# slowkow/scde

Measured on AMD Instinct MI355X. Metric: genes/sec for scde.expression.difference (400-pt grid, 100 randomizations), higher is better.
Workload: dtype f64; 1 GPU; config3: synthetic 20000 genes x 1000 cells (500/500), 401-pt grid, 100 bootstraps, n.cores=1 seeding; genes_total=20000, genes_per_gpu=20000, cells=1000, grid=401, n_randomizations=100, parallelism=gene-shard x1 (strong)

## Files before the change

scde_amd/csrc/engine.hip:

```cpp
#include <hip/hip_runtime.h>

#include <algorithm>
#include <chrono>
#include <cfloat>
#include <cmath>
#include <cerrno>
#include <cstdarg>
#include <cstdio>
#include <cstdlib>
#include <cstring>
#include <condition_variable>
#include <deque>
#include <functional>
#include <thread>
#include <atomic>
#include <memory>
#include <unistd.h>
#include <mutex>
#include <numeric>
#include <string>
#include <vector>

#include "engine_internal.h"
#include "kernels.h"
// ... 691 lines not shown
      pu.into_col0 = col0;
      pu.into_c0 = c0;
      pu.into_cap_hint = c0 > 0 ? (long long)((double)col0 / c0 * C * 1.1) : 0;
      const PostSpec* sp[1] = {&ps};
      UniqueSet* up[1] = {&pu};
      const hipStream_t main = cx->stream;
      cx->stream = s.piece_stream;
      const int rc = build_unique_sets(cx, sp, up, 1);
      cx->stream = main;
      pu.into = nullptr;
      RCHK(rc);
      HCHK(handoff_spin(cx, s.piece_stream));
      HCHK(hipEventRecord(s.piece_ev[j], s.piece_stream));
      HCHK(handoff_wait(cx, st, s.piece_ev[j]));
      for (int c = c0; c < c1; ++c) ucl_off_h[c + 1] = col0 + pu.ucl_off_h[c - c0 + 1];
      const long long nc = pu.ucl_off_h[c1 - c0];
      if (j == jlast) RCHK(upload(cx, u.ucl_off, ucl_off_h.data(), sizeof(long long) * (C + 1)));
      const long long est = std::max<long long>(col0 + nc, (long long)((double)(col0 + nc) / c1 * C * 1.1));
      RCHK(setup_tables(plan0, est, j > 0));
      RCHK(launch_tables_range(plan0, c0, c1, col0, pu.ucl_off.as<long long>(), pu.ucl_off_h, j == jlast, pu));
      if (modes_pieces) {
        HCHK(launch_modes(u.uci.as<int>() + (size_t)N * c0, N, N, c1 - c0, pu.ucl_off.as<long long>(),
                          cx->maxi.as<int>() + col0, cx->mag.as<double>(), s.modes + (size_t)N * c0, 1, N, st));
        const size_t bytes = sizeof(double) * (size_t)N * (c1 - c0);
        RCHK(dnl_push(cx, st, s.modes_host + (size_t)N * c0, bytes, s.modes + (size_t)N * c0, bytes, bytes, 1));
      }
      col0 += nc;
    }
    ta.ucl_off = u.ucl_off.as<long long>();
    tables_done = make_plan(col0) == plan0;
  }
  const long long ncols = ucl_off_h[C];
  const Plan plan = make_plan(ncols);
  const bool fast = plan.fast, fused = plan.fused, stretch_skip = plan.stretch_skip;
  bool tpath = plan.tpath;
  ta.ncols = ncols;
  if (!tables_done) {
    if (plan.tpath && !plan0.tpath) {
      HCHK(cx->qflags.ensure(sizeof(int) * 40));
      HCHK(hipMemsetAsync(cx->qflags.p, 0, sizeof(int) * 40, st));
    }
    if (plan.fused) {
      HCHK(cx->base_col.ensure(sizeof(int) * std::max(1, C)));
      HCHK(cx->zcol.ensure(sizeof(int) * std::max(1, C)));
    }
    RCHK(setup_tables(plan, ncols, false));
    ta.ncols = ncols;
    RCHK(launch_tables_range(plan, 0, C, 0, u.ucl_off.as<long long>(), ucl_off_h, true, cx->task_us));
  }
  std::vector<int> draws;
  std::vector<double> W;
  int ndraw = 0, maxw = 0;
  const int nsets = (int)s.seeds.size();
  const int qstride = (int)round_up(std::max(Cmax, 1), 64) + 64;
  int nb = fast ? boot2_nb(s.nboot) : 16;
  if (fast) {
    const int v = cx->opt_boot_nb;
    if (v >= 4 && v <= 32 && v % 4 == 0) nb = v;
  }
  const int Bp = (int)round_up(std::max(s.nboot, 1), nb);
  const int Bt = (int)round_up(Bp, 32) + 128;
  auto rest_fn = [=, &s, &u]() mutable -> int {
  if (want_modes && s.modes && s.modes_early && !modes_pieces) {
    HCHK(launch_modes(u.uci.as<int>(), N, N, C, u.ucl_off.as<long long>(), cx->maxi.as<int>(),
                      cx->mag.as<double>(), s.modes, 1, N, st));
    if (s.modes_host) {
      const size_t bytes = sizeof(double) * (size_t)N * C;
      RCHK(dnl_push(cx, st, s.modes_host, bytes, s.modes, bytes, bytes, 1));
    } else {
      if (!cx->modes_ev) HCHK(hipEventCreateWithFlags(&cx->modes_ev, hipEventDisableTiming));
      HCHK(handoff_spin(cx, st));
      HCHK(hipEventRecord(cx->modes_ev, st));
    }
  }
  bool jp_sent = false;
  const bool dev_mult = fused && C <= kMultMaxCells;
  if (fused && s.nboot > 0) {
    if (dev_mult) {
      make_draws(s, Bp, draws, W, ndraw, &maxw, false);
    } else {
      make_draws(s, Bp, draws, W, ndraw);
      maxw = 0;
      for (double w : W) maxw = std::max(maxw, (int)w);
    }
    tpath = tpath && maxw <= std::min(127, cx->opt_tile_max_mult);
  }
  if (!s.batch_call && s.ensemble) {
    HCHK(cx->E.ensure(sizeof(double) * std::max<long long>(1, ncols) * GS));
    HCHK(launch_ensemble_cols(cx->T.as<double>(), ncols, G, GS, cx->E.as<double>(), st));
    NoBootArgs na{cx->E.as<double>(), G, GS, u.ucl_off.as<long long>(), u.uci.as<int>(), N, C, N, 1,
                  s.jp, s.jp_g, s.jp_k};
    HCHK(launch_noboot(na, st));
  } else if (s.nboot == 0 && !s.batch_call) {
    NoBootArgs na{cx->T.as<double>(), G, GS, u.ucl_off.as<long long>(), u.uci.as<int>(), N, C, N, 0,
                  s.jp, s.jp_g, s.jp_k};
    HCHK(launch_noboot(na, st));
  } else if (s.nboot == 0) {
    HCHK(hipMemsetAsync(s.jp, 0, sizeof(double) * (size_t)N * G, st));
  } else {
    if (!fused) make_draws(s, Bp, draws, W, ndraw);
    hipStream_t sa = st;
    if (fused) {
      if (!cx->aux_stream) HCHK(hipStreamCreateWithFlags(&cx->aux_stream, hipStreamNonBlocking));
      if (!cx->aux_ev) HCHK(hipEventCreateWithFlags(&cx->aux_ev, hipEventDisableTiming));
      sa = cx->aux_stream;
      HCHK(handoff_wait(cx, sa, cx->p1_ev));
// ... 1938 lines not shown
```

scde_amd/csrc/kernels.h:

```cpp
#pragma once

#ifndef SCDE_BOOT_WPE
#define SCDE_BOOT_WPE 8
#endif
#ifndef SCDE_BOOT_ASMLD
#define SCDE_BOOT_ASMLD 1
#endif
#ifndef SCDE_TAB_WPE
#define SCDE_TAB_WPE 4
#endif
#ifndef SCDE_BOOT_EB
#define SCDE_BOOT_EB 4
#endif
#ifndef SCDE_BOOT_DIAG
#define SCDE_BOOT_DIAG 0
#endif
#ifndef SCDE_RATIO_WPE
#define SCDE_RATIO_WPE 1
#endif
#ifndef SCDE_RATIO_DIAG
#define SCDE_RATIO_DIAG 0
#endif
#ifndef SCDE_WPCA_BLOCK
#define SCDE_WPCA_BLOCK 512
// ... 133 lines not shown
  const long long* ucl_off;
  const int* uci;
  long long ld_uci;
  double norm_mult;
  const int* degen;
  double* out;
  long long out_g, out_k;
  int ngenes;
  int g_lo = 0, g_hi = -1;
};

struct NoBootArgs {
  const double* T;
  int G, GS;
  const long long* ucl_off;
  const int* uci;
  long long ld_uci;
  int ncells, ngenes;
  int ensemble;
  double* out;
  long long out_g, out_k;
};

struct RatioArgs {
  const double* jp1;
  long long j1g, j1k;
  const double* jp2;
  long long j2g, j2k;
  const double* prior_y;
  int n, ngenes;
  int normalize;
  const double* xin;
  long long xg, xo;
  double* ratio;
  long long rg, ro;
  const double* diffv;
  int zi;
  double* res;
  long long res_ld;
};

hipError_t launch_cell_prep(const double* models, int ncells, int G, int GS, const double* mag, int lt, int sq,
                            double* mu, double* lcfp, double* lcfpr, double* theta, double* cellscal,
                            double* pq, hipStream_t s, double* cfp = nullptr);
hipError_t launch_col_consts(const int* ucl, const long long* ucl_off, long long ncols, int ncells,
                             const double* theta, int GS, const double* cellscal, double* colc, hipStream_t s);
hipError_t launch_tables(const TablesArgs& a, hipStream_t s);
hipError_t launch_stretch_zu(const double* U, const int* base_col, int ncells, const double* Wt, int Bp, int nsets,
                             double* ZU, hipStream_t s, int gsets = 0, int gsplit = 0);
hipError_t launch_base_cols(const int* ucl, const long long* ucl_off, int ncells, const unsigned char* has_clamp,
                            int use_baseline, int* base_col, hipStream_t s);
hipError_t launch_widen16(const unsigned short* in, int* out, size_t n, hipStream_t s);
hipError_t launch_patch32(const int2* exc, size_t n, int* out, hipStream_t s);
hipError_t launch_ell(const int* uci, long long ld_uci, int ngenes, int ncells, const long long* ucl_off,
                      const int* base_col, int stride, int pad_col, int padto, int2* ent, int* nnz, hipStream_t s,
                      int cell_off, const int* ucl = nullptr, unsigned* key = nullptr, int* idx = nullptr,
                      int kg0 = 0, int kgn = 0, int kch = 1, int desc = 0);
hipError_t launch_baseline_z(const double* T, int G, int GS, const int* base_col, int ncells, const double* Wt,
                             int Bp, int nsets, double* Z, hipStream_t s, int gsets = 0, int gsplit = 0);
constexpr int kMultMaxCells = 16384;
hipError_t launch_mult(const int* draws, int nsets, int nboot, int ndraw, int ncells, int Bp, double* Wt, int Bt,
                       unsigned char* W8, int nb, int P, unsigned char* W8p, int SG, int NGR, unsigned char* W8g,
                       hipStream_t s);
hipError_t launch_spin(hipStream_t s, long long cycles);
hipError_t launch_boot(const BootArgs& a, hipStream_t s);
hipError_t launch_boot_exact(const ExactArgs& a, hipStream_t s);
int boot2_nb(int nboot);
hipError_t launch_boot2(const Boot2Args& a, hipStream_t s);
hipError_t launch_delta(const double* T, const long long* ucl_off, int ncells, long long ncols, const int* base_col,
                        int G, int GS, double* D, hipStream_t s);
hipError_t launch_noboot(const NoBootArgs& a, hipStream_t s);
hipError_t launch_ensemble_cols(const double* T, long long ncols, int G, int GS, double* E, hipStream_t s);
hipError_t launch_modes(const int* uci, long long ld_uci, int ngenes, int ncells, const long long* ucl_off,
                        const int* maxi, const double* mag, double* modes, long long mg, long long mc,
                        hipStream_t s);
hipError_t launch_post(const int* uci, long long ld_uci, int ngenes, int c, const long long* ucl_off,
                       const double* T, int G, int GS, double* post, long long pg, long long pk, hipStream_t s);
hipError_t launch_cell_minmax(const int* counts, long long ld, long long g0, int ngenes, int ncells,
                              const int* cellidx, int* cmax, int* cmin, hipStream_t s);
hipError_t launch_mark(const int* counts, long long ld, long long g0, int ngenes, int ncells, const int* cellidx,
                       const long long* woff, unsigned long long* bits, hipStream_t s,
                       int* flags = nullptr);
hipError_t launch_rank(const unsigned long long* bits, const long long* woff, int ncells, int* rank, int* nuniq,
                       hipStream_t s,
                       const int* flags_in = nullptr, int* flags_out = nullptr);
hipError_t launch_fill_ucl(const unsigned long long* bits, const long long* woff, int ncells, const int* rank,
                           const long long* ucl_off, int* ucl, hipStream_t s);
hipError_t launch_uci(const int* counts, long long ld, long long g0, int ngenes, int ncells, const int* cellidx,
                      const long long* woff, const unsigned long long* bits, const int* rank, int* uci,
                      hipStream_t s);
hipError_t launch_colmajor_to_rows(const double* src, int nrows, int ncols, int GS, double* dst, hipStream_t s);
hipError_t launch_bh_cz(const double* z, int n, double* cz, void* work, size_t* work_bytes, hipStream_t s);

hipError_t launch_prior_stats(const int* counts, long long ld, int N, int C, const double* cellp, int sq,
                              double* vout, int* occ, double* partials, int nb, double* out, hipStream_t s);
long long prior_items(int N, int C);
int prior_blocks(int N, int C, int cap);
int prior_grid_n(int L);
hipError_t launch_prior_bin(const int* counts, long long ld, int N, int C, const double* cellp, int sq,
                            const int* occ, double wsum, double max_value, double bw, int L,
                            unsigned long long* hist, int nb, hipStream_t s);
hipError_t launch_prior_tail(double tot_mass, double max_value, double bw, int L, double pc,
                             const unsigned long long* hist, double* work, double* out, hipStream_t s);
hipError_t launch_sort_doubles(const double* in, double* out, long long n, void* work, size_t* work_bytes,
                               hipStream_t s);
hipError_t launch_ratio_summary(const RatioArgs& a, hipStream_t s);
// ... 172 lines not shown
```

scde_amd/csrc/kernels.hip:

```cpp
#include <hip/hip_runtime.h>
#include <algorithm>
#include <cmath>
#include <cstdint>
#include <utility>

#include "device_math.h"
#include "kernels.h"
#include "wave_ops.h"

namespace scde {

__global__ __launch_bounds__(256) void k_cell_prep(const double* __restrict__ models, int ncells, int G, int GS,
                                                   const double* __restrict__ mag, int localtheta,
                                                   int squarelogit, double* __restrict__ mu,
                                                   double* __restrict__ lcfp, double* __restrict__ lcfpr,
                                                   double* __restrict__ theta, double* __restrict__ cellscal,
                                                   double* __restrict__ pq, double* __restrict__ cfpo) {
  const int c = blockIdx.x;
  auto M = [&](int col) { return models[(long long)c + (long long)ncells * col]; };
  const double concb = M(0), conca = M(1), failr = M(2), corrb = M(3), corra = M(4), corrt = M(5);
  const double ltb = M(6), ltt = M(7), ltm = M(8), lts = M(9), ltr = M(10), conca2 = M(11);
  double lmax = -INFINITY;
  for (int k = threadIdx.x; k < G; k += blockDim.x) {
    const double m = mag[k];
// ... 1676 lines not shown
    const unsigned qv[16] = {q0.x, q0.y, q0.z, q0.w, q1.x, q1.y, q1.z, q1.w,
                             q2.x, q2.y, q2.z, q2.w, q3.x, q3.y, q3.z, q3.w};
#pragma unroll
    for (int tt = 0; tt < 16; ++tt) sq[tt * 64 + lane] = qv[tt];
    const unsigned wv[8] = {w0.x, w0.y, w0.z, w0.w, w1.x, w1.y, w1.z, w1.w};
    unsigned short* sw16 = reinterpret_cast<unsigned short*>(sw);
#pragma unroll
    for (int j = 0; j < 8; ++j) {
      sw16[(2 * j) * 64 + lane] = (unsigned short)(wv[j] & 0xffffu);
      sw16[(2 * j + 1) * 64 + lane] = (unsigned short)(wv[j] >> 16);
    }
    wave_sync();
    const uint4* bq = reinterpret_cast<const uint4*>(sq + t * 64 + 16 * h);
    const uint4 b0v = bq[0], b1v = bq[1], b2v = bq[2], b3v = bq[3];
    const unsigned u[16] = {b0v.x, b0v.y, b0v.z, b0v.w, b1v.x, b1v.y, b1v.z, b1v.w,
                            b2v.x, b2v.y, b2v.z, b2v.w, b3v.x, b3v.y, b3v.z, b3v.w};
    const uint4* aw = reinterpret_cast<const uint4*>(sw + r * 32 + 8 * h);
    const uint4 a0v = aw[0], a1v = aw[1];
    const unsigned x2[8] = {a0v.x, a0v.y, a0v.z, a0v.w, a1v.x, a1v.y, a1v.z, a1v.w};
    i32x4 af[2];
    unsigned lo4[4], hi4[4];
#pragma unroll
    for (int q = 0; q < 4; ++q) {
      lo4[q] = __builtin_amdgcn_perm(x2[2 * q + 1], x2[2 * q], 0x06040200u);
      hi4[q] = __builtin_amdgcn_perm(x2[2 * q + 1], x2[2 * q], 0x07050301u);
    }
    af[0] = i32x4{(int)lo4[0], (int)lo4[1], (int)lo4[2], (int)lo4[3]};
    af[1] = i32x4{(int)hi4[0], (int)hi4[1], (int)hi4[2], (int)hi4[3]};
    unsigned pl[4][4];
#pragma unroll
    for (int q = 0; q < 4; ++q)
      tr4(u[4 * q], u[4 * q + 1], u[4 * q + 2], u[4 * q + 3], pl[0][q], pl[1][q], pl[2][q], pl[3][q]);
#pragma unroll
    for (int l = 0; l < 4; ++l) {
      const i32x4 bf = {(int)pl[l][0], (int)pl[l][1], (int)pl[l][2], (int)pl[l][3]};
      acc[0][l] = mfma_i8(af[0], bf, acc[0][l]);
      acc[1][l] = mfma_i8(af[1], bf, acc[1][l]);
    }
  }
  if (t < NTB)
#pragma unroll
    for (int bt = 0; bt < 2; ++bt)
#pragma unroll
      for (int q = 0; q < 4; ++q) {
        const int b = 16 * bt + 4 * h + q;
        if (b < nbout) {
          const long long v =
              (((long long)acc[bt][3][q] * 256 + acc[bt][2][q]) * 256 + acc[bt][1][q]) * 256 + acc[bt][0][q];
          atomicAdd(reinterpret_cast<unsigned long long*>(&dsum[t * 32 + b]), (unsigned long long)v);
        }
      }
}

template <int NB>
__device__ __forceinline__ void tile_rows(double (&a0)[NB], double (&a1)[NB], const double* __restrict__ D,
                                          const int2* __restrict__ E, int n, const double* __restrict__ W,
                                          const double* __restrict__ Zs, int GS, int Bp, int b0, int k0, int r,
                                          bool live, bool l0, bool l1) {
#pragma unroll
  for (int i = 0; i < NB; ++i) {
    const d2_t z = live ? *reinterpret_cast<const d2_t*>(Zs + (long long)(b0 + i) * GS + k0) : d2_t{0.0, 0.0};
    a0[i] = l0 ? z.x : -INFINITY;
    a1[i] = l1 ? z.y : -INFINITY;
  }
  {
    constexpr int EB2 = 2;
    const unsigned doff = (unsigned)k0 * 8u;
    const unsigned woff = (unsigned)(b0 + 2 * min(r, NB / 2 - 1)) * 8u;
    d2_t v[EB2], vb[EB2], w[EB2], wb[EB2];
    auto fetch = [&](int e0, int4& t) { t = *reinterpret_cast<const int4*>(E + e0); };
    const int col0 = __builtin_amdgcn_readfirstlane(E[0].y);
    (void)col0;
    auto issue = [&](int4 t, d2_t (&x)[EB2], d2_t (&wv)[EB2]) {
      asm volatile("" : "+s"(t.x), "+s"(t.y), "+s"(t.z), "+s"(t.w));
      const double* d0 = D + (unsigned)(((SCDE_TILE_DIAG & 8) ? col0 : t.y) * GS);
      const double* d1 = D + (unsigned)(((SCDE_TILE_DIAG & 8) ? col0 : t.w) * GS);
      const double* w0 = W + (unsigned)(t.x * Bp);
      const double* w1 = W + (unsigned)(t.z * Bp);
      asm volatile("global_load_dwordx4 %0, %1, %2" : "=v"(x[0]) : "v"(doff), "s"(d0));
      if (!(SCDE_TILE_DIAG & 4)) asm volatile("global_load_dwordx4 %0, %1, %2" : "=v"(wv[0]) : "v"(woff), "s"(w0));
      asm volatile("global_load_dwordx4 %0, %1, %2" : "=v"(x[1]) : "v"(doff), "s"(d1));
      if (!(SCDE_TILE_DIAG & 4)) asm volatile("global_load_dwordx4 %0, %1, %2" : "=v"(wv[1]) : "v"(woff), "s"(w1));
    };
    auto ready = [&](d2_t (&x)[EB2], d2_t (&wv)[EB2]) {
      if (SCDE_TILE_DIAG & 4)
        asm volatile("s_waitcnt vmcnt(2)" : "+v"(x[0]), "+v"(x[1]), "+v"(wv[0]), "+v"(wv[1]));
      else
        asm volatile("s_waitcnt vmcnt(4)" : "+v"(x[0]), "+v"(x[1]), "+v"(wv[0]), "+v"(wv[1]));
    };
    auto accumulate = [&](const d2_t (&x)[EB2], const d2_t (&wv)[EB2]) {
#pragma unroll
      for (int j = 0; j < EB2; ++j)
        fmac_entry2<NB>(a0, a1, wv[j], x[j], std::make_integer_sequence<int, NB / 2>{});
    };
#pragma unroll
    for (int i = 0; i < NB; ++i) asm volatile("" : "+v"(a0[i]), "+v"(a1[i]));
    int4 ta, tb;
    fetch(0, ta);
    if (SCDE_TILE_DIAG & 4) {
      const double* w0 = W + (unsigned)(ta.x * Bp);
      w[0] = w[1] = wb[0] = wb[1] = *reinterpret_cast<const d2_t*>(w0 + woff / 8);
      asm volatile("s_waitcnt vmcnt(0)" : "+v"(w[0]), "+v"(w[1]), "+v"(wb[0]), "+v"(wb[1]));
    }
    issue(ta, v, w);
    fetch(EB2, tb);
    const int n2 = (n + EB2 - 1) & ~(EB2 - 1);
    int e0 = 0;
    for (; e0 + 2 * EB2 <= n2; e0 += 2 * EB2) {
      issue(tb, vb, wb);
      fetch(e0 + 2 * EB2, ta);
      ready(v, w);
      accumulate(v, w);
      issue(ta, v, w);
      fetch(e0 + 3 * EB2, tb);
      ready(vb, wb);
      accumulate(vb, wb);
    }
    if (e0 < n2) {
      issue(tb, vb, wb);
      ready(v, w);
      accumulate(v, w);
      asm volatile("s_waitcnt vmcnt(0)" : "+v"(vb[0]), "+v"(vb[1]), "+v"(wb[0]), "+v"(wb[1]));
    }
    asm volatile("s_waitcnt vmcnt(0)" : "+v"(v[0]), "+v"(v[1]), "+v"(w[0]), "+v"(w[1]));
  }
}

template <int NB, int WB>
__global__ __launch_bounds__(64 * WB) __attribute__((amdgpu_waves_per_eu(SCDE_TILE_WPE))) void k_boot_tiles(
    const double* __restrict__ D, const int2* __restrict__ ent, const int* __restrict__ nnz, int ent_stride,
    const double* __restrict__ Wt, int Bp, int ncells, const int* __restrict__ wset, const double* __restrict__ Z,
    int G, int GS, int P, int nboot, double norm_mult, double degen_thresh, double* __restrict__ part,
    long long part_stride, int* __restrict__ degen, int ngenes, const unsigned char* __restrict__ W8p, int Bq,
    const unsigned* __restrict__ UQ, const int* __restrict__ ZUq, const int* __restrict__ nanflag, int maxgroups,
    int* __restrict__ redo, int* __restrict__ stats, unsigned* __restrict__ pmask,
    const int* __restrict__ slab_list) {
  static_assert(NB % 4 == 0 && NB <= 20, "NB must be a multiple of 4, <= 20");
  __shared__ float ubs[WB][kBTileMax * NB];
#ifdef SCDE_TILE_TEST_WB1
  __shared__ unsigned bstage[WB][64];
#else
  __shared__ unsigned bstage[WB][1024 + 512];
#endif
  __shared__ float fmx[WB][32];
  __shared__ double etab[64];
  const int lane = threadIdx.x & 63;
  const int wsid = __builtin_amdgcn_readfirstlane(threadIdx.x >> 6);
  if (xcd_block(blockIdx.x, gridDim.x) * WB >= slab_list[0]) return;
  if (threadIdx.x < 64) etab[threadIdx.x] = kExp2Frac64[threadIdx.x];
  __syncthreads();
#ifndef SCDE_TILE_TEST_WB1
  static_assert(2 * (8 * NB + NB) <= (int)(sizeof(bstage[0]) / 4),
                "the staging area must hold the tile sums and the normalisers");
#endif
  double* const tsum = reinterpret_cast<double*>(&bstage[wsid][0]);
  double* const finv = tsum + 8 * NB;
  const int idx = xcd_block(blockIdx.x, gridDim.x) * WB + wsid;
  if (idx >= slab_list[0]) return;
  const int it = slab_list[1 + idx];
  const int g = it / P, p = it - g * P;
  if (*nanflag) {
    if (lane == 0) {
      const int q = (long long)g * P + p;
      redo[q] = 1;
      redo[(long long)ngenes * P + 1 + atomicAdd(&redo[(long long)ngenes * P], 1)] = q;
      pmask[q] = ~0u;
    }
    return;
  }
  const int n = nnz[g];
  const int NT = (G + 15) >> 4, NTB = (G + 31) >> 5;
  const int r = lane & 15;
  const int2* __restrict__ E = ent + (long long)g * ent_stride;
  const int set = wset ? wset[g] : 0;
  const int b0 = p * NB;
  {
    const unsigned pstride = 32u * (unsigned)P;
    const unsigned char* __restrict__ W8 = W8p + (long long)set * ncells * pstride + 32 * p;
    const int* __restrict__ ZU = ZUq + (long long)set * 4 * kQTiles * Bq + b0;
    tile_bound_pass(E, n, UQ, W8, pstride, ZU, Bq, &bstage[wsid][0], ubs[wsid], NB, NB, NTB, lane);
  }
  wave_sync();
  const int nlive = min(NB, nboot - b0);
  float sc = -INFINITY;
  if (lane < NTB)
    for (int b = 0; b < nlive; ++b) sc = fmaxf(sc, ubs[wsid][lane * NB + b]);
  const int nsel = min(max(1, min(maxgroups, 4)), NTB);
  int tl[4] = {0, 0, 0, 0};
  unsigned bd = 0;
#pragma unroll
  for (int j = 0; j < 4; ++j) {
    if (j < nsel) {
      float m = sc;
      m = fmaxf(m, dpp_f<kDppXor1>(m));
      m = fmaxf(m, dpp_f<kDppXor2>(m));
      m = fmaxf(m, dpp_f<kDppHalfMirror>(m));
      m = fmaxf(m, dpp_f<kDppMirror>(m));
      m = __int_as_float(__builtin_amdgcn_readfirstlane(__float_as_int(m)));
      const unsigned long long bl = __ballot(lane < NTB && !((bd >> lane) & 1) && sc == m);
      const int t = __ffsll((long long)bl) - 1;
      tl[j] = t;
      bd |= 1u << t;
      if (lane == t) sc = -INFINITY;
    }
  }
  const unsigned ntmask = (NT >= 32) ? ~0u : ((1u << NT) - 1);
  unsigned done = 0;
#pragma unroll
  for (int j = 0; j < 4; ++j)
    if (j < nsel) done |= 3u << (2 * tl[j]);
  done &= ntmask;
  const int slot = lane >> 3, m2 = lane & 7, row = lane >> 4;
  int mybt = tl[0];
#pragma unroll
  for (int j = 1; j < 4; ++j) mybt = (row == j) ? tl[j] : mybt;
  const int mytile = 2 * mybt + (slot & 1);
  const int k0 = 16 * mytile + 2 * m2;
  const bool live = row < nsel;
  const bool l0 = live && k0 < G, l1 = live && k0 + 1 < G;
  const double* __restrict__ W = Wt + (long long)set * ncells * Bp;
  const double* __restrict__ Zs = Z + (long long)set * Bp * GS;
  double a0[NB], a1[NB];
  tile_rows<NB>(a0, a1, D, E, n, W, Zs, GS, Bp, b0, k0, r, live, l0, l1);
  {
    double mx[NB];
#pragma unroll
    for (int i = 0; i < NB; ++i) mx[i] = gt_max(a0[i], a1[i]);
    wave_max_partials_all<NB>(mx, &fmx[0][0], lane, wsid);
  }
  wave_sync();
  bool need = false;
  if (lane < NTB && !((bd >> lane) & 1))
    for (int b = 0; b < nlive; ++b) need |= (double)ubs[wsid][lane * NB + b] >= (double)fmx[wsid][b] - 51.0;
  const bool fail = __ballot(need) != 0;
  if (fail && lane == 0) {
    const int q = g * P + p;
    redo[q] = 1;
    redo[(long long)ngenes * P + 1 + atomicAdd(&redo[(long long)ngenes * P], 1)] = q;
    pmask[q] = ~0u;
    if (stats) {
      atomicAdd(&stats[3], 1);
      atomicAdd(&stats[5], (n + 3) & ~3);
    }
  }
  if (stats && lane == 0) atomicAdd(&stats[4], 2 * ((n + 1) & ~1));
  if (fail) return;
  if (lane == 0)
    for (int b = 0; b < nlive; ++b)
      if (!(fabs((double)fmx[wsid][b]) <= degen_thresh)) degen[g] = 1;
#pragma unroll
  for (int i = 0; i < NB; ++i) {
    const double m = (double)fmx[wsid][i];
    const double d0 = a0[i] - m, d1 = a1[i] - m;
    const bool n0 = l0 && d0 >= kBootExpCut, n1 = l1 && d1 >= kBootExpCut;
    if (__builtin_amdgcn_ballot_w64(n0 || n1)) {
      a0[i] = n0 ? exp_tab(d0, etab) : 0.0;
      a1[i] = n1 ? exp_tab(d1, etab) : 0.0;
    } else {
      a0[i] = 0.0;
      a1[i] = 0.0;
    }
    const double ps = pair8_sum(a0[i], a1[i]);
    if (m2 == 0 && live) tsum[slot * NB + i] = ps;
  }
  wave_sync();
  if (lane < NB) {
    double S = 0.0;
    for (unsigned mm = done; mm; mm &= mm - 1) {
      const int t = __builtin_ffs((int)mm) - 1;
      int sslot = 0;
#pragma unroll
      for (int j = 0; j < 4; ++j)
        if (tl[j] == (t >> 1) && j < nsel) sslot = 2 * j + (t & 1);
      S += tsum[sslot * NB + lane];
    }
    finv[lane] = (b0 + lane < nboot) ? 1.0 / (S * norm_mult) : 0.0;
// ... 21 lines not shown
      atomicAdd(&stats[6 + __builtin_popcount(done)], 1);
    }
  }
}

template <int N, int CTRL>
__device__ __forceinline__ void row_halve_f(float (&v)[32], bool up) {
  constexpr int H = (N + 1) / 2;
#pragma unroll
  for (int j = 0; j < H; ++j) {
    const float lo = v[j], hi = (j + H < N) ? v[j + H] : -INFINITY;
    v[j] = gt_maxf(up ? hi : lo, dpp_f<CTRL>(up ? lo : hi));
  }
}
template <int N>
__device__ __forceinline__ void row_max_scatter_f(float (&v)[32], int r) {
  constexpr int H1 = (N + 1) / 2, H2 = (H1 + 1) / 2, H3 = (H2 + 1) / 2;
  row_halve_f<N, kDppMirror>(v, (r & 8) != 0);
  row_halve_f<H1, kDppHalfMirror>(v, (r & 4) != 0);
  row_halve_f<H2, kDppXor2>(v, (r & 2) != 0);
  row_halve_f<H3, kDppXor1>(v, (r & 1) != 0);
}
template <int N>
__device__ __forceinline__ int row_scatter_index(int r, int j) {
  constexpr int H1 = (N + 1) / 2, H2 = (H1 + 1) / 2, H3 = (H2 + 1) / 2, H4 = (H3 + 1) / 2;
  const int p4 = j + H4 * (r & 1), p3 = p4 + H3 * ((r >> 1) & 1), p2 = p3 + H2 * ((r >> 2) & 1),
            p1 = p2 + H1 * ((r >> 3) & 1);
  return (j < H4 && p4 < H3 && p3 < H2 && p2 < H1 && p1 < N) ? p1 : -1;
}

template <int N, int CTRL>
__device__ __forceinline__ void pair_halve(double (&v)[32], bool up) {
  constexpr int H = (N + 1) / 2;
#pragma unroll
  for (int j = 0; j < H; ++j) {
    const double lo = v[j], hi = (j + H < N) ? v[j + H] : 0.0;
    v[j] = (up ? hi : lo) + dpp_d<CTRL>(up ? lo : hi);
  }
}
template <int N>
__device__ __forceinline__ void pair4_scatter(double (&v)[32], int m) {
  constexpr int H1 = (N + 1) / 2;
  pair_halve<N, kDppXor1>(v, (m & 1) != 0);
  pair_halve<H1, kDppXor2>(v, (m & 2) != 0);
}
template <int N>
__device__ __forceinline__ int pair_scatter_index(int m, int j) {
  constexpr int H1 = (N + 1) / 2, H2 = (H1 + 1) / 2;
  const int p2 = j + H2 * ((m >> 1) & 1), p1 = p2 + H1 * (m & 1);
  return (j < H2 && p2 < H1 && p1 < N) ? p1 : -1;
}

constexpr int kGeneSlabs = 8;
template <int NB, int WB>
__global__ __launch_bounds__(64 * WB) __attribute__((amdgpu_waves_per_eu(SCDE_TILE_WPE))) void k_boot_gene(
    const double* __restrict__ D, const int2* __restrict__ ent, const int* __restrict__ nnz, int ent_stride,
    const double* __restrict__ Wt, int Bp, int ncells, const int* __restrict__ wset, const double* __restrict__ Z,
    int G, int GS, int P, int SG, int nboot, double norm_mult, double degen_thresh, double* __restrict__ part,
    long long part_stride, int* __restrict__ degen, int ngenes, const unsigned char* __restrict__ W8g, int Bq,
    const unsigned* __restrict__ UQ, const int* __restrict__ ZUq, const int* __restrict__ nanflag, int maxgroups,
    int kcap, int* __restrict__ redo, int* __restrict__ stats, const int* __restrict__ order,
    unsigned* __restrict__ pmask, int* __restrict__ wide, int wide_cap, int blk0, double* __restrict__ out,
    long long out_g, long long out_k, int* __restrict__ gdone) {
  static_assert(NB % 4 == 0 && NB <= 20, "NB must be a multiple of 4, <= 20");
  static_assert(WB == 3 || WB == 4, "3 or 4 waves per gene block");
  constexpr int kGeneRows = 4 * WB;
  __shared__ unsigned bstage[WB][1024 + 512];
  __shared__ long long dsum[WB < 4 ? kBTileMax * 32 : 1];
  __shared__ float gub[kBTileMax * 128];
  __shared__ float sc[kGeneSlabs][16];
  __shared__ signed char rk[kGeneSlabs][16];
  __shared__ signed char rowof[kGeneSlabs][16];
  __shared__ int rowS[kGeneRows], rowT[kGeneRows];
  __shared__ double fmx[kGeneSlabs][32];
  __shared__ unsigned bd[kGeneSlabs];
  __shared__ unsigned failm;
  __shared__ double etab[64];
  static_assert(kGeneRows * 32 + 2 * (4 * kGeneRows * NB) + 2 * kGeneSlabs * 32 <= WB * (1024 + 512),
                "the staging area must hold the row maxima, tile sums and normalisers");
  float* const rowmax = reinterpret_cast<float*>(&bstage[0][0]);
  double* const tsum = reinterpret_cast<double*>(&bstage[0][0] + kGeneRows * 32);
  double* const finv = tsum + 4 * kGeneRows * NB;
  const int lane = threadIdx.x & 63;
  const int wsid = __builtin_amdgcn_readfirstlane(threadIdx.x >> 6);
  const int NGR = (P + SG - 1) / SG;
  const int blk = blk0 + xcd_block(blockIdx.x, gridDim.x);
  if (blk >= ngenes * NGR) return;
  const int gi = blk / NGR, gr = blk - gi * NGR;
  const int g = order ? order[gi] : gi;
  const int s0 = gr * SG, ns = min(SG, P - s0);
  const bool direct = gdone && NGR == 1 && ns * ((G + 31) & ~31) * 8 <= (int)sizeof(bstage);
  if (gdone && threadIdx.x == 0) gdone[g] = 0;
  if (*nanflag) {
    if ((int)threadIdx.x < ns) {
      const int q = g * P + s0 + threadIdx.x;
      redo[q] = 1;
      redo[(long long)ngenes * P + 1 + atomicAdd(&redo[(long long)ngenes * P], 1)] = q;
      pmask[q] = ~0u;
    }
    return;
  }
  if (threadIdx.x < 64) etab[threadIdx.x] = kExp2Frac64[threadIdx.x];
  if (threadIdx.x == 0) failm = 0u;
  if (WB < 4) {
    for (int i = threadIdx.x; i < kBTileMax * 32; i += 64 * WB) dsum[i] = 0;
    __syncthreads();
  }
  const int n = nnz[g];
// ... 36 lines not shown
      float v = -INFINITY;
      if (s < ns && t < NTB) {
        const int nl = min(NB, nboot - (gb0 + s * NB));
        for (int b = 0; b < nl; ++b) v = fmaxf(v, gub[t * 128 + s * NB + b]);
      }
      sc[s][t] = v;
      rowof[s][t] = -1;
    } else if (s < kGeneSlabs + 1 && t < kGeneRows) {
      rowS[t] = -1;
      rowT[t] = 0;
    }
  }
  __syncthreads();
  {
    const int s = threadIdx.x >> 4, t = threadIdx.x & 15;
    if (s < ns && t < NTB) {
      const float v = sc[s][t];
      int rnk = 0;
      for (int u = 0; u < NTB; ++u) {
        const float w = sc[s][u];
        rnk += (w > v) || (w == v && u < t);
      }
      rk[s][rnk] = (signed char)t;
    }
  }
  __syncthreads();
  const int K = min(min(4, kGeneRows / ns), min(NTB, max(1, min(maxgroups, kcap))));
  {
    const int x = threadIdx.x;
    if (x < K * ns) {
      const int s = x / K;
      rowS[x] = s;
      rowT[x] = rk[s][x - s * K];
    } else if (x >= 64 && x < 64 + 2 * ns && maxgroups >= 4 && kcap >= 4) {
      const int c = x - 64, s = c >> 1, k = K + (c & 1);
      const int nsp = kGeneRows - K * ns;
      if (k < NTB && nsp > 0) {
        const float key = sc[s][rk[s][k]] - sc[s][rk[s][0]];
        int o = 0;
        for (int c2 = 0; c2 < 2 * ns; ++c2) {
          const int s2 = c2 >> 1, k2 = K + (c2 & 1);
          if (k2 >= NTB) continue;
          const float key2 = sc[s2][rk[s2][k2]] - sc[s2][rk[s2][0]];
          o += (key2 > key) || (key2 == key && c2 < c);
        }
        if (o < nsp) {
          rowS[K * ns + o] = s;
          rowT[K * ns + o] = rk[s][k];
        }
      }
    }
  }
  __syncthreads();
  const int row = lane >> 4, q = 4 * wsid + row;
  const int sq = rowS[q];
  const bool live = sq >= 0;
  const int tq = live ? rowT[q] : 0;
  const int slot = lane >> 3, m2 = lane & 7, r = lane & 15;
  const int k0 = 16 * (2 * tq + (slot & 1)) + 2 * m2;
  const bool l0 = live && k0 < G, l1 = live && k0 + 1 < G;
  const int b0 = gb0 + (live ? sq : 0) * NB;
  const double* __restrict__ W = Wt + (long long)set * ncells * Bp;
  const double* __restrict__ Zs = Z + (long long)set * Bp * GS;
  double a0[NB], a1[NB];
  if (SCDE_TILE_DIAG & 32) {
#pragma unroll
    for (int i = 0; i < NB; ++i) {
      a0[i] = l0 ? (double)(k0 + i) : -INFINITY;
      a1[i] = l1 ? (double)(k0 + i) : -INFINITY;
    }
  } else {
    tile_rows<NB>(a0, a1, D, E, n, W, Zs, GS, Bp, b0, k0, r, live, l0, l1);
  }
  if (SCDE_TILE_DIAG & 64) {
    double v = 0.0;
#pragma unroll
    for (int i = 0; i < NB; ++i) v += a0[i] + a1[i];
    if (v == 12345.0) part[0] = v;
    return;
  }
  if (!(SCDE_TILE_DIAG & 2048)) {
    float v[32];
#pragma unroll
    for (int i = 0; i < NB; ++i) v[i] = (float)gt_max(a0[i], a1[i]);
    row_max_scatter_f<NB>(v, r);
#pragma unroll
    for (int j = 0; j < 2; ++j) {
      const int idx = row_scatter_index<NB>(r, j);
      if (idx >= 0) rowmax[q * 32 + idx] = v[j];
    }
  }
  __syncthreads();
  {
    for (int x = threadIdx.x; x < ns * 32; x += 64 * WB) {
      const int s = x >> 5, i = x & 31;
      if (i < NB) {
        float m = -INFINITY;
        if (SCDE_TILE_DIAG & 2048) {
          m = 0.0f;
        } else {
          for (int j = 0; j < K; ++j) m = gt_maxf(m, rowmax[(s * K + j) * 32 + i]);
          for (int q2 = K * ns; q2 < kGeneRows; ++q2)
            if (rowS[q2] == s) m = gt_maxf(m, rowmax[q2 * 32 + i]);
        }
        fmx[s][i] = m;
      }
    }
    if ((int)threadIdx.x < ns) {
      const int s = threadIdx.x;
      unsigned b = 0;
      for (int q2 = s * K; q2 < s * K + K; ++q2) {
        b |= 1u << rowT[q2];
        rowof[s][rowT[q2]] = (signed char)q2;
      }
      for (int q2 = K * ns; q2 < kGeneRows; ++q2)
        if (rowS[q2] == s) {
          b |= 1u << rowT[q2];
          rowof[s][rowT[q2]] = (signed char)q2;
        }
      bd[s] = b;
    }
  }
  __syncthreads();
  for (int s = wsid; s < ns; s += WB) {
    const int nl = min(NB, nboot - (gb0 + s * NB));
    const int tt = lane & 15;
// ... 534 lines not shown
```

scde_amd/csrc/unique.hip:

```cpp
#include <hip/hip_runtime.h>
#include <algorithm>
#include <cmath>
#include <cstdint>

#include "kernels.h"

namespace scde {

__global__ void k_cell_minmax(const int* __restrict__ counts, long long ld, long long g0, int ngenes,
                              const int* __restrict__ cellidx, int* __restrict__ cmax, int* __restrict__ cmin) {
  __shared__ int smax[16], smin[16];
  const int c = blockIdx.x;
  const int* col = counts + (long long)cellidx[c] * ld + g0;
  int mx = 0, mn = 0x7fffffff;
  const int head = (int)min<long long>(ngenes, (4 - (((uintptr_t)col >> 2) & 3)) & 3);
  const int nv = (ngenes - head) >> 2;
  const int4* col4 = reinterpret_cast<const int4*>(col + head);
  for (int i = threadIdx.x; i < nv; i += blockDim.x) {
    const int4 x = col4[i];
    mx = max(mx, max(max(x.x, x.y), max(x.z, x.w)));
    mn = min(mn, min(min(x.x, x.y), min(x.z, x.w)));
  }
  for (int g = threadIdx.x; g < head; g += blockDim.x) {
    mx = max(mx, col[g]);
// ... 180 lines not shown
  for (int c0 = 0; c0 < ncells; c0 += 64) {
    __syncthreads();
#pragma unroll
    for (int r = 0; r < RPW; ++r) tile[wid + r * kEllWaves][lane] = pu[r];
    const long long off = poff;
    const int bc = pbc;
    __syncthreads();
    if (c0 + 64 < ncells) prefetch(c0 + 64);
    const int c = c0 + lane;
#pragma unroll
    for (int i = 0; i < GPW; ++i) {
      const int gl = wid * GPW + i, g = g0 + gl;
      if (g >= ngenes) break;
      int col = -1;
      bool keep = false;
      if (c < ncells) {
        col = (int)(off + tile[lane][gl]);
        keep = col != bc;
      }
      const unsigned long long m = __ballot(keep);
      const int pos = n[i] + __builtin_amdgcn_mbcnt_hi((unsigned)(m >> 32), __builtin_amdgcn_mbcnt_lo((unsigned)m, 0));
      if (keep) ent[(long long)g * stride + pos] = make_int2(c + cell_off, col);
      if (want_key && keep) ks[i] += (unsigned)max(ucl[col], 0);
      n[i] += __popcll(m);
    }
  }
#pragma unroll
  for (int i = 0; i < GPW; ++i) {
    const int g = g0 + wid * GPW + i;
    if (g >= ngenes) break;
    unsigned long long kv = ks[i];
    if (want_key) {
#pragma unroll
      for (int o = 32; o >= 1; o >>= 1) kv += __shfl_xor(kv, o, 64);
    }
    const int nn = n[i];
    if (lane == 0) {
      nnz[g] = nn;
      if (want_key) {
        const long long gg = (long long)kg0 + g;
        int k = (int)(gg * kch / kgn);
        while (k + 1 < kch && (long long)kgn * (k + 1) / kch <= gg) ++k;
        while (k > 0 && (long long)kgn * k / kch > gg) --k;
        int hb = 0;
        while ((1 << hb) < kch) ++hb;
        const unsigned vmax = (1u << (kEllKeyBits - hb)) - 1u;
        unsigned v = (unsigned)(log2((double)kv + 1.0) * ((double)vmax / 33.0));
        v = v > vmax ? vmax : v;
        if (desc) v = vmax - v;
        key[g] = (hb ? ((unsigned)k << (kEllKeyBits - hb)) : 0u) | v;
        idx[g] = kg0 + g;
      }
    }
    const int end = padto == 64 ? (nn > 0 ? (nn + 63) & ~63 : 64) + 8 : ((nn + 7) & ~7) + 8;
    int2* E = ent + (long long)g * stride;
    for (int q = nn + lane; q < end && q < stride; q += 64) E[q] = make_int2(0, pad_col);
  }
}

__global__ void k_modes(const int* __restrict__ uci, long long ld_uci, int ngenes, int ncells,
                        const long long* __restrict__ ucl_off, const int* __restrict__ maxi,
                        const double* __restrict__ mag, double* __restrict__ modes, long long mg, long long mc) {
  const long long i = (long long)blockIdx.x * blockDim.x + threadIdx.x;
  if (i >= (long long)ngenes * ncells) return;
  const int g = (int)(i % ngenes), c = (int)(i / ngenes);
  const long long col = ucl_off[c] + uci[(long long)g + ld_uci * c];
  modes[g * mg + c * mc] = mag[maxi[col]];
}

__global__ void k_post(const int* __restrict__ uci, long long ld_uci, int ngenes, int c,
                       const long long* __restrict__ ucl_off, const double* __restrict__ T, int G, int GS,
                       double* __restrict__ post, long long pg, long long pk) {
  const long long i = (long long)blockIdx.x * blockDim.x + threadIdx.x;
  if (i >= (long long)ngenes * G) return;
  const int g = (int)(i % ngenes), k = (int)(i / ngenes);
  const long long col = ucl_off[c] + uci[(long long)g + ld_uci * c];
  post[g * pg + k * pk] = T[col * GS + k];
}

__global__ void k_colmajor_to_rows(const double* __restrict__ src, int nrows, int ncols, int GS,
                                   double* __restrict__ dst) {
  const long long i = (long long)blockIdx.x * blockDim.x + threadIdx.x;
  if (i >= (long long)nrows * ncols) return;
  const int r = (int)(i % nrows), k = (int)(i / nrows);
  dst[(long long)r * GS + k] = src[i];
}

__global__ void k_spin(long long cycles) {
  const long long t0 = clock64();
  while (clock64() - t0 < cycles) __builtin_amdgcn_s_sleep(1);
}

hipError_t launch_spin(hipStream_t s, long long cycles) {
  if (cycles <= 0) return hipSuccess;
  hipLaunchKernelGGL(k_spin, dim3(1), dim3(64), 0, s, std::min(cycles, 100000000LL));
  return hipGetLastError();
}

hipError_t launch_patch32(const int2* exc, size_t n, int* out, hipStream_t s) {
  if (n == 0) return hipSuccess;
  hipLaunchKernelGGL(k_patch32, dim3((unsigned)div_up((long long)n, 256)), dim3(256), 0, s, exc, (long long)n, out);
  return hipGetLastError();
}

hipError_t launch_widen16(const unsigned short* in, int* out, size_t n, hipStream_t s) {
  if (n == 0) return hipSuccess;
  hipLaunchKernelGGL(k_widen16, dim3((unsigned)div_up((long long)n, 256)), dim3(256), 0, s, in, out, (long long)n);
  return hipGetLastError();
}

hipError_t launch_ell(const int* uci, long long ld_uci, int ngenes, int ncells, const long long* ucl_off,
                      const int* base_col, int stride, int pad_col, int padto, int2* ent, int* nnz, hipStream_t s,
                      int cell_off, const int* ucl, unsigned* key, int* idx, int kg0, int kgn, int kch, int desc) {
  if (ngenes <= 0) return hipSuccess;
  if (padto == 64 ? stride < ((ncells + 63) & ~63) + 8 || stride < 72 : stride < ((ncells + 7) & ~7) + 8)
    return hipErrorInvalidValue;
  if (cell_off < 0) return hipErrorInvalidValue;
  if (key && (!ucl || !idx || kch < 1 || kgn < kg0 + ngenes || kch > kgn)) return hipErrorInvalidValue;
  hipLaunchKernelGGL(k_ell, dim3(div_up(ngenes, 64)), dim3(64 * kEllWaves), 0, s, uci, ld_uci, ngenes, ncells, ucl_off,
                     base_col, stride, pad_col, padto, ent, nnz, cell_off, ucl, key, idx, kg0, kgn, kch, desc);
  return hipGetLastError();
}

hipError_t launch_modes(const int* uci, long long ld_uci, int ngenes, int ncells, const long long* ucl_off,
                        const int* maxi, const double* mag, double* modes, long long mg, long long mc,
                        hipStream_t s) {
  const long long n = (long long)ngenes * ncells;
  if (n <= 0) return hipSuccess;
  hipLaunchKernelGGL(k_modes, dim3(div_up(n, 256)), dim3(256), 0, s, uci, ld_uci, ngenes, ncells, ucl_off, maxi,
                     mag, modes, mg, mc);
  return hipGetLastError();
}

hipError_t launch_post(const int* uci, long long ld_uci, int ngenes, int c, const long long* ucl_off,
                       const double* T, int G, int GS, double* post, long long pg, long long pk, hipStream_t s) {
  const long long n = (long long)ngenes * G;
  if (n <= 0) return hipSuccess;
  hipLaunchKernelGGL(k_post, dim3(div_up(n, 256)), dim3(256), 0, s, uci, ld_uci, ngenes, c, ucl_off, T, G, GS,
                     post, pg, pk);
  return hipGetLastError();
}

hipError_t launch_cell_minmax(const int* counts, long long ld, long long g0, int ngenes, int ncells,
                              const int* cellidx, int* cmax, int* cmin, hipStream_t s) {
  if (ncells <= 0) return hipSuccess;
  hipLaunchKernelGGL(k_cell_minmax, dim3(ncells), dim3(256), 0, s, counts, ld, g0, ngenes, cellidx, cmax, cmin);
  return hipGetLastError();
}

hipError_t launch_mark(const int* counts, long long ld, long long g0, int ngenes, int ncells, const int* cellidx,
                       const long long* woff, unsigned long long* bits, hipStream_t s, int* flags) {
  const long long n = (long long)ngenes * ncells;
  if (n <= 0) return hipSuccess;
  hipLaunchKernelGGL((k_mark<8, 16>), dim3(div_up(ngenes, 256 * 8), ncells), dim3(256), 0, s, counts, ld, g0,
                     ngenes, cellidx, woff, bits, flags);
  return hipGetLastError();
}

hipError_t launch_rank(const unsigned long long* bits, const long long* woff, int ncells, int* rank, int* nuniq,
                       hipStream_t s, const int* flags_in, int* flags_out) {
  if (ncells <= 0) return hipSuccess;
  hipLaunchKernelGGL(k_rank, dim3(ncells), dim3(256), 0, s, bits, woff, rank, nuniq, flags_in, flags_out);
  return hipGetLastError();
}

hipError_t launch_fill_ucl(const unsigned long long* bits, const long long* woff, int ncells, const int* rank,
                           const long long* ucl_off, int* ucl, hipStream_t s) {
  if (ncells <= 0) return hipSuccess;
// ... 23 lines not shown
```

Before: 3.156 million genes/s.

## Generalize tile_rows load pipeline to a configurable-depth ring buffer

Replaces the hard-coded double-buffered gather/weight prefetch in tile_rows with a templated ring of depth LA, parameterizing vmcnt waits. The ELL pad grows to cover the deeper lookahead, and k_boot_gene gets its own waves-per-EU macro and recomputes its lane-row constants after the tile loop to shorten register live ranges. The defaults (LA=2, WPE=4) keep the same ring depth as before, so the main behavioural changes are the waves-per-EU setting on k_boot_gene and the register-pressure restructuring. A deeper ring would raise the number of loads in flight at the cost of more VGPRs.

```diff
diff --git a/scde_amd/csrc/engine.hip b/scde_amd/csrc/engine.hip
--- a/scde_amd/csrc/engine.hip
+++ b/scde_amd/csrc/engine.hip
@@ -767,6 +767,7 @@
   std::vector<double> W;
   int ndraw = 0, maxw = 0;
   const int nsets = (int)s.seeds.size();
+  static_assert(kEllTilePad <= 64, "the row stride's 64 spare entries must hold the ELL pad");
   const int qstride = (int)round_up(std::max(Cmax, 1), 64) + 64;
   int nb = fast ? boot2_nb(s.nboot) : 16;
   if (fast) {
diff --git a/scde_amd/csrc/kernels.h b/scde_amd/csrc/kernels.h
--- a/scde_amd/csrc/kernels.h
+++ b/scde_amd/csrc/kernels.h
@@ -209,6 +209,8 @@
                             int use_baseline, int* base_col, hipStream_t s);
 hipError_t launch_widen16(const unsigned short* in, int* out, size_t n, hipStream_t s);
 hipError_t launch_patch32(const int2* exc, size_t n, int* out, hipStream_t s);
+constexpr int kTileRingMax = 4;
+constexpr int kEllTilePad = 2 * kTileRingMax;
 hipError_t launch_ell(const int* uci, long long ld_uci, int ngenes, int ncells, const long long* ucl_off,
                       const int* base_col, int stride, int pad_col, int padto, int2* ent, int* nnz, hipStream_t s,
                       int cell_off, const int* ucl = nullptr, unsigned* key = nullptr, int* idx = nullptr,
diff --git a/scde_amd/csrc/kernels.hip b/scde_amd/csrc/kernels.hip
--- a/scde_amd/csrc/kernels.hip
+++ b/scde_amd/csrc/kernels.hip
@@ -1752,11 +1752,13 @@
       }
 }
 
-template <int NB>
+template <int NB, int LA>
 __device__ __forceinline__ void tile_rows(double (&a0)[NB], double (&a1)[NB], const double* __restrict__ D,
                                           const int2* __restrict__ E, int n, const double* __restrict__ W,
                                           const double* __restrict__ Zs, int GS, int Bp, int b0, int k0, int r,
                                           bool live, bool l0, bool l1) {
+  static_assert(LA >= 2 && 2 * LA <= kEllTilePad, "the ring's furthest fetch must stay inside the ELL row's pad");
+  static_assert(4 * LA <= 63, "loads in flight must fit the 6-bit vmcnt");
 #pragma unroll
   for (int i = 0; i < NB; ++i) {
     const d2_t z = live ? *reinterpret_cast<const d2_t*>(Zs + (long long)(b0 + i) * GS + k0) : d2_t{0.0, 0.0};
@@ -1767,7 +1769,7 @@
     constexpr int EB2 = 2;
     const unsigned doff = (unsigned)k0 * 8u;
     const unsigned woff = (unsigned)(b0 + 2 * min(r, NB / 2 - 1)) * 8u;
-    d2_t v[EB2], vb[EB2], w[EB2], wb[EB2];
+    d2_t v[LA][EB2], w[LA][EB2];
     auto fetch = [&](int e0, int4& t) { t = *reinterpret_cast<const int4*>(E + e0); };
     const int col0 = __builtin_amdgcn_readfirstlane(E[0].y);
     (void)col0;
@@ -1784,9 +1786,13 @@
     };
     auto ready = [&](d2_t (&x)[EB2], d2_t (&wv)[EB2]) {
       if (SCDE_TILE_DIAG & 4)
-        asm volatile("s_waitcnt vmcnt(2)" : "+v"(x[0]), "+v"(x[1]), "+v"(wv[0]), "+v"(wv[1]));
+        asm volatile("s_waitcnt vmcnt(%4)" : "+v"(x[0]), "+v"(x[1]), "+v"(wv[0]), "+v"(wv[1]) : "n"(EB2 * (LA - 1)));
       else
-        asm volatile("s_waitcnt vmcnt(4)" : "+v"(x[0]), "+v"(x[1]), "+v"(wv[0]), "+v"(wv[1]));
+        asm volatile("s_waitcnt vmcnt(%4)" : "+v"(x[0]), "+v"(x[1]), "+v"(wv[0]), "+v"(wv[1])
+                     : "n"(2 * EB2 * (LA - 1)));
+    };
+    auto landed = [&](d2_t (&x)[EB2], d2_t (&wv)[EB2]) {
+      asm volatile("s_waitcnt vmcnt(0)" : "+v"(x[0]), "+v"(x[1]), "+v"(wv[0]), "+v"(wv[1]));
     };
     auto accumulate = [&](const d2_t (&x)[EB2], const d2_t (&wv)[EB2]) {
 #pragma unroll
@@ -1795,34 +1801,39 @@
     };
 #pragma unroll
     for (int i = 0; i < NB; ++i) asm volatile("" : "+v"(a0[i]), "+v"(a1[i]));
-    int4 ta, tb;
-    fetch(0, ta);
+    int4 t[LA];
+    fetch(0, t[0]);
     if (SCDE_TILE_DIAG & 4) {
-      const double* w0 = W + (unsigned)(ta.x * Bp);
-      w[0] = w[1] = wb[0] = wb[1] = *reinterpret_cast<const d2_t*>(w0 + woff / 8);
-      asm volatile("s_waitcnt vmcnt(0)" : "+v"(w[0]), "+v"(w[1]), "+v"(wb[0]), "+v"(wb[1]));
-    }
-    issue(ta, v, w);
-    fetch(EB2, tb);
+      const double* w0 = W + (unsigned)(t[0].x * Bp);
+#pragma unroll
+      for (int j = 0; j < LA; ++j) {
+        w[j][0] = w[j][1] = *reinterpret_cast<const d2_t*>(w0 + woff / 8);
+        asm volatile("s_waitcnt vmcnt(0)" : "+v"(w[j][0]), "+v"(w[j][1]));
+      }
+    }
+#pragma unroll
+    for (int j = 0; j < LA - 1; ++j) {
+      issue(t[j], v[j], w[j]);
+      fetch(EB2 * (j + 1), t[j + 1]);
+    }
+    auto step = [&](int e, int j) {
+      const int jn = (j + LA - 1) % LA;
+      issue(t[jn], v[jn], w[jn]);
+      fetch(e + EB2 * LA, t[j]);
+      ready(v[j], w[j]);
+      accumulate(v[j], w[j]);
+    };
     const int n2 = (n + EB2 - 1) & ~(EB2 - 1);
     int e0 = 0;
-    for (; e0 + 2 * EB2 <= n2; e0 += 2 * EB2) {
-      issue(tb, vb, wb);
-      fetch(e0 + 2 * EB2, ta);
-      ready(v, w);
-      accumulate(v, w);
-      issue(ta, v, w);
-      fetch(e0 + 3 * EB2, tb);
-      ready(vb, wb);
-      accumulate(vb, wb);
-    }
-    if (e0 < n2) {
-      issue(tb, vb, wb);
-      ready(v, w);
-      accumulate(v, w);
-      asm volatile("s_waitcnt vmcnt(0)" : "+v"(vb[0]), "+v"(vb[1]), "+v"(wb[0]), "+v"(wb[1]));
-    }
-    asm volatile("s_waitcnt vmcnt(0)" : "+v"(v[0]), "+v"(v[1]), "+v"(w[0]), "+v"(w[1]));
+    for (; e0 + LA * EB2 <= n2; e0 += LA * EB2) {
+#pragma unroll
+      for (int j = 0; j < LA; ++j) step(e0 + EB2 * j, j);
+    }
+#pragma unroll
+    for (int j = 0; j < LA - 1; ++j)
+      if (e0 + EB2 * j < n2) step(e0 + EB2 * j, j);
+#pragma unroll
+    for (int j = LA - 1; j >= 0; --j) landed(v[j], w[j]);
   }
 }
 
@@ -1921,7 +1932,7 @@
   const double* __restrict__ W = Wt + (long long)set * ncells * Bp;
   const double* __restrict__ Zs = Z + (long long)set * Bp * GS;
   double a0[NB], a1[NB];
-  tile_rows<NB>(a0, a1, D, E, n, W, Zs, GS, Bp, b0, k0, r, live, l0, l1);
+  tile_rows<NB, 2>(a0, a1, D, E, n, W, Zs, GS, Bp, b0, k0, r, live, l0, l1);
   {
     double mx[NB];
 #pragma unroll
@@ -2049,8 +2060,14 @@
 }
 
 constexpr int kGeneSlabs = 8;
+#ifndef SCDE_GENE_WPE
+#define SCDE_GENE_WPE 4
+#endif
+#ifndef SCDE_GENE_LA
+#define SCDE_GENE_LA 2
+#endif
 template <int NB, int WB>
-__global__ __launch_bounds__(64 * WB) __attribute__((amdgpu_waves_per_eu(SCDE_TILE_WPE))) void k_boot_gene(
+__global__ __launch_bounds__(64 * WB) __attribute__((amdgpu_waves_per_eu(SCDE_GENE_WPE))) void k_boot_gene(
     const double* __restrict__ D, const int2* __restrict__ ent, const int* __restrict__ nnz, int ent_stride,
     const double* __restrict__ Wt, int Bp, int ncells, const int* __restrict__ wset, const double* __restrict__ Z,
     int G, int GS, int P, int SG, int nboot, double norm_mult, double degen_thresh, double* __restrict__ part,
@@ -2193,26 +2210,42 @@
     }
   }
   __syncthreads();
-  const int row = lane >> 4, q = 4 * wsid + row;
-  const int sq = rowS[q];
-  const bool live = sq >= 0;
-  const int tq = live ? rowT[q] : 0;
-  const int slot = lane >> 3, m2 = lane & 7, r = lane & 15;
-  const int k0 = 16 * (2 * tq + (slot & 1)) + 2 * m2;
-  const bool l0 = live && k0 < G, l1 = live && k0 + 1 < G;
-  const int b0 = gb0 + (live ? sq : 0) * NB;
-  const double* __restrict__ W = Wt + (long long)set * ncells * Bp;
-  const double* __restrict__ Zs = Z + (long long)set * Bp * GS;
+  struct RowLane {
+    int q, sq, tq, slot, m2, r, k0;
+    bool live, l0, l1;
+  };
+  auto row_lane = [&](int ln) {
+    RowLane c;
+    c.q = 4 * wsid + (ln >> 4);
+    c.sq = rowS[c.q];
+    c.live = c.sq >= 0;
+    c.tq = c.live ? rowT[c.q] : 0;
+    c.slot = ln >> 3, c.m2 = ln & 7, c.r = ln & 15;
+    c.k0 = 16 * (2 * c.tq + (c.slot & 1)) + 2 * c.m2;
+    c.l0 = c.live && c.k0 < G, c.l1 = c.live && c.k0 + 1 < G;
+    return c;
+  };
   double a0[NB], a1[NB];
-  if (SCDE_TILE_DIAG & 32) {
-#pragma unroll
-    for (int i = 0; i < NB; ++i) {
-      a0[i] = l0 ? (double)(k0 + i) : -INFINITY;
-      a1[i] = l1 ? (double)(k0 + i) : -INFINITY;
-    }
-  } else {
-    tile_rows<NB>(a0, a1, D, E, n, W, Zs, GS, Bp, b0, k0, r, live, l0, l1);
-  }
+  {
+    const RowLane c = row_lane(lane);
+    const int b0 = gb0 + (c.live ? c.sq : 0) * NB;
+    const double* __restrict__ W = Wt + (long long)set * ncells * Bp;
+    const double* __restrict__ Zs = Z + (long long)set * Bp * GS;
+    if (SCDE_TILE_DIAG & 32) {
+#pragma unroll
+      for (int i = 0; i < NB; ++i) {
+        a0[i] = c.l0 ? (double)(c.k0 + i) : -INFINITY;
+        a1[i] = c.l1 ? (double)(c.k0 + i) : -INFINITY;
+      }
+    } else {
+      tile_rows<NB, SCDE_GENE_LA>(a0, a1, D, E, n, W, Zs, GS, Bp, b0, c.k0, c.r, c.live, c.l0, c.l1);
+    }
+  }
+  int lane_again = lane;
+  asm volatile("" : "+v"(lane_again));
+  const RowLane c = row_lane(lane_again);
+  const int q = c.q, sq = c.sq, slot = c.slot, m2 = c.m2, r = c.r, k0 = c.k0;
+  const bool live = c.live, l0 = c.l0, l1 = c.l1;
   if (SCDE_TILE_DIAG & 64) {
     double v = 0.0;
 #pragma unroll
diff --git a/scde_amd/csrc/unique.hip b/scde_amd/csrc/unique.hip
--- a/scde_amd/csrc/unique.hip
+++ b/scde_amd/csrc/unique.hip
@@ -256,7 +256,7 @@
         idx[g] = kg0 + g;
       }
     }
-    const int end = padto == 64 ? (nn > 0 ? (nn + 63) & ~63 : 64) + 8 : ((nn + 7) & ~7) + 8;
+    const int end = padto == 64 ? (nn > 0 ? (nn + 63) & ~63 : 64) + kEllTilePad : ((nn + 7) & ~7) + 8;
     int2* E = ent + (long long)g * stride;
     for (int q = nn + lane; q < end && q < stride; q += 64) E[q] = make_int2(0, pad_col);
   }
@@ -317,7 +317,8 @@
                       const int* base_col, int stride, int pad_col, int padto, int2* ent, int* nnz, hipStream_t s,
                       int cell_off, const int* ucl, unsigned* key, int* idx, int kg0, int kgn, int kch, int desc) {
   if (ngenes <= 0) return hipSuccess;
-  if (padto == 64 ? stride < ((ncells + 63) & ~63) + 8 || stride < 72 : stride < ((ncells + 7) & ~7) + 8)
+  if (padto == 64 ? stride < ((ncells + 63) & ~63) + kEllTilePad || stride < 64 + kEllTilePad
+                  : stride < ((ncells + 7) & ~7) + 8)
     return hipErrorInvalidValue;
   if (cell_off < 0) return hipErrorInvalidValue;
   if (key && (!ucl || !idx || kch < 1 || kgn < kg0 + ngenes || kch > kgn)) return hipErrorInvalidValue;
```

Result: no change. 3.135 million genes/s (-0.7%).
